# talmolab/Brax-Rodent-Run

Hardware: AMD Instinct MI355X
Metric: env-steps/sec (whole node), rodent 2048 envs/GPU (higher is better)
Workload: dtype f32

## Files before the change

### brax-rodent-run_amd/csrc/rr_api.hip

```cpp
#include "../../include/rodent_rr.h"
#include "rr_kernel.h"
#include "rr_mlp.h"
#include "rr_ppo.h"

#include <atomic>
#include <climits>
#include <cstdio>
#include <cstdlib>
#include <cstring>
#include <map>
#include <memory>
#include <mutex>
#include <string>
#include <type_traits>
#include <vector>

static thread_local std::string g_err;
static int fail(int code, const std::string& msg) { g_err = msg; return code; }
extern "C" const char* rr_last_error(void) { return g_err.c_str(); }

#define HIPCHK(x)                                                                                  \
  do {                                                                                             \
    hipError_t e_ = (x);                                                                           \
    if (e_ != hipSuccess) return fail(RR_EHIP, std::string(#x) + ": " + hipGetErrorString(e_));   \
// ... 99 lines not shown
  m->dbg_names.clear(); m->dbg_off.clear(); m->dbg_size.clear(); m->dbg_cnames.clear();
  m->stage_ok = stage_fits(d.nbody, d.nv, con_slots, k.nalias);
  if (m->dyn && d.nu > std::max(7 * d.nbody + 4, 6 * d.nv)) m->stage_ok = false;
  int g = 0;
  auto dbg = [&](const char* name, int n) { int r = g; m->dbg_names.push_back(name); m->dbg_off.push_back(g); m->dbg_size.push_back(n); g += n; return r; };
  k.g_xpos = dbg("xpos", 3 * d.nbody); k.g_xquat = dbg("xquat", 4 * d.nbody); k.g_xmat = dbg("xmat", 9 * d.nbody);
  k.g_com = dbg("subtree_com", 6); k.g_cinert = dbg("cinert", 10 * d.nbody); k.g_crb = dbg("crb", 10 * d.nbody);
  k.g_cdof = dbg("cdof", 6 * d.nv); k.g_cvel = dbg("cvel", 6 * d.nbody); k.g_cfrc = dbg("cfrc", 6 * d.nbody);
  k.g_qM = dbg("qM", d.nM); k.g_qLD = dbg("qLD", d.nM); k.g_dinv = dbg("qLDiagInv", d.nv);
  k.g_bias = dbg("qfrc_bias", d.nv); k.g_passive = dbg("qfrc_passive", d.nv); k.g_actuator = dbg("qfrc_actuator", d.nv);
  k.g_smooth = dbg("qfrc_smooth", d.nv); k.g_qacc_smooth = dbg("qacc_smooth", d.nv);
  k.g_con_dist = dbg("con_dist", d.ncon); k.g_con_pos = dbg("con_pos", 3 * d.ncon); k.g_con_frame = dbg("con_frame", 9 * d.ncon);
  k.g_con_D = dbg("con_D", d.ncon); k.g_con_aref = dbg("con_aref", 4 * d.ncon); k.g_lim = dbg("limit_pos_D_aref", 3 * d.nv);
  k.g_qacc = dbg("qacc", d.nv); k.g_qfrc_constraint = dbg("qfrc_constraint", d.nv); k.g_misc = dbg("niter_cost", 2);
  k.g_ls_iters = dbg("ls_iters", 2);
  k.g_kaok = dbg("kernarg_ok", 1);
  k.dbg_floats = g;
  for (auto& s : m->dbg_names) m->dbg_cnames.push_back(s.c_str());
  m->dims.lds_bytes = L.lds_floats * (int)sizeof(float);
  m->dims.dbg_floats = g;
  m->dims.solver = m->solver;
  m->dims.fixed_instance = select(m, F_STEP, V_PROD).fixed ? 1 : 0;
}

static void setup_replica(rr_model* m) {
  m->pair_ok = false;
  const char* sw = getenv("RR_PAIR_WAVES");
  if (sw && sw[0] == '0') return;
  static const char* need[] = {"h_dims", "h_k_slots", "h_k_body_i", "h_k_body_f", "h_k_jnt_i", "h_k_jnt_f", "h_k_dof_i", "h_k_dof_f", "h_k_act_f", "h_k_M_ij_k",
                               "h_k_body_anc", "h_k_nround", "h_k_factor3", "h_k_factor3_rows", "h_k_linv", "h_k_linv_rows", "h_k_coljob", "h_k_rowjob", "h_k_jobown",
// ... 149 lines not shown
  RRTables T_rep;
  std::vector<void*> dev_allocs;
  bool timing = false;
  std::vector<hipEvent_t> ev0, ev1;
  int npending = 0, ring_head = 0;
  double total_ms = 0;
  int64_t launches = 0;
  unsigned long long* prof = nullptr;
  const int32_t* env_map = nullptr;
  uint32_t* cost = nullptr;
  bool counted = false;
  unsigned* dyn_overflow = nullptr;
  unsigned* bad_states = nullptr;
  unsigned* progress = nullptr;
  float *env_dof_f = nullptr, *env_act_f = nullptr, *env_con_f = nullptr;
  int ls_run_repeats = 0;
  float* eval_actions = nullptr;
  bool has_env_params() const { return env_dof_f || env_act_f || env_con_f; }
};

template <typename Ptr>
static int dev_alloc(rr_batch* b, size_t bytes, Ptr* dst, const void* host = nullptr, size_t host_bytes = 0) {
  void* p = nullptr;
  HIPCHK(hipMalloc(&p, bytes));
  b->dev_allocs.push_back(p);
  if (host_bytes) HIPCHK(hipMemcpy(p, host, host_bytes, hipMemcpyHostToDevice));
  *dst = (Ptr)p;
  return RR_OK;
}
template <typename Ptr>
static int upload(rr_batch* b, const char* name, Ptr* dst) {
// ... 228 lines not shown
  if (rc) return rc;
  HIPCHK(hipSetDevice(b->device));
  const rr_model* m = b->m;
  const bool geom = io.o_cdist || io.o_cpos || io.o_cframe, params = b->has_env_params();
  if (params && io.dbg) return fail(RR_EUNSUPPORTED, "launch: no debug dump on a batch with per-env parameters (the debug instance reads the model's shared tables)");
  if (params && geom) return fail(RR_EUNSUPPORTED, "launch: no contact-geometry outputs on a batch with per-env parameters (they are served by the debug instance)");
  if (params && b->prof) return fail(RR_EUNSUPPORTED, "launch: no profile build on a batch with per-env parameters");
  Variant v = b->prof ? V_PROFILE : ((io.dbg || geom) ? V_DEBUG : (params ? V_RAND : V_PROD));
  const bool pair = m->pair_ok && v == V_PROD && !L.env && !L.out && !L.un && !b->env_map && !b->cost && m->solver != 2;
  if (pair) v = V_PAIR;
  const Instance in = select(m, L.ev ? F_EVAL : (L.ac ? F_ACTOR : (L.un ? F_UNROLL : F_STEP)), v);
  if (!in.kern) return fail(RR_EUNSUPPORTED, std::string(L.un ? "" : "launch: ") + in.why);
  if (L.un && (rc = fill_unroll(b, L, io))) return rc;
  io.env_dof_f = b->env_dof_f; io.env_act_f = b->env_act_f; io.env_con_f = b->env_con_f;
  io.prof = b->prof; io.env_map = b->env_map; io.cost = b->cost; io.dyn_overflow = b->dyn_overflow; io.bad_states = b->bad_states;
  if (v == V_DEBUG) io.ls_run_repeats = b->ls_run_repeats;
  RRDims kd = pair ? m->kd_rep : b->kd;
  kd.iterations = m->kd.iterations; kd.ls_iterations = m->kd.ls_iterations;
  if (b->timing) {
    if (b->npending == RR_TIMING_RING && (rc = collect_timing(b, false))) return rc;
    HIPCHK(hipEventRecord(b->ev0[(b->ring_head + b->npending) % RR_TIMING_RING], b->stream));
  }
  hipLaunchKernelGGL(in.kern, dim3(b->N), dim3((pair ? 2 : 1) * RR_LANES), (size_t)lds_bytes(m, v), b->stream, kd, pair ? b->T_rep : b->T, io, b->N, L.n_frames);
  HIPCHK(hipGetLastError());
  if (b->timing) {
    HIPCHK(hipEventRecord(b->ev1[(b->ring_head + b->npending) % RR_TIMING_RING], b->stream));
    b->npending += 1;
  }
  return RR_OK;
}

// ... 632 lines not shown
    *own[i] = (float*)q;
    HIPCHK(hipMemcpyAsync(q, src[i], bytes[i], hipMemcpyDeviceToDevice, b->stream));
  }
  HIPCHK(hipStreamSynchronize(b->stream));
  return RR_OK;
}

extern "C" int rr_batch_set_schedule(rr_batch* b, const int32_t* env_map, uint32_t* cost_cycles) {
  if (!b) return fail(RR_EINVAL, "rr_batch_set_schedule: null batch");
  b->env_map = env_map; b->cost = cost_cycles;
  return RR_OK;
}

extern "C" int rr_batch_set_ls_repeat_exit(rr_batch* b, int32_t enable) {
  if (!b) return fail(RR_EINVAL, "rr_batch_set_ls_repeat_exit: null batch");
  b->ls_run_repeats = enable ? 0 : 1;
  return RR_OK;
}

extern "C" int rr_batch_set_timing(rr_batch* b, int32_t enable) {
  if (!b) return fail(RR_EINVAL, "rr_batch_set_timing: null batch");
  HIPCHK(hipSetDevice(b->device));
  if (enable && b->ev0.empty()) {
    for (int i = 0; i < RR_TIMING_RING; ++i) {
      hipEvent_t a, c;
      HIPCHK(hipEventCreate(&a)); b->ev0.push_back(a);
      HIPCHK(hipEventCreate(&c)); b->ev1.push_back(c);
    }
  }
  b->timing = enable != 0;
  b->total_ms = 0; b->launches = 0; b->npending = 0; b->ring_head = 0;
// ... 11 lines not shown
```

### brax-rodent-run_amd/csrc/rr_kernel.h

```cpp
#pragma once
#include <hip/hip_runtime.h>
#include <stdint.h>
#include "rr_tanh_normal.h"

#define RR_LANES 64
#define RR_DOFI 12
#define RR_BODYI 12
#ifndef RR_WIDE
#define RR_WIDE 1
#endif
#ifndef RR_RING
#define RR_RING 6
#endif

#define RR_NPH 24
#ifndef RR_W1
#define RR_W1 2
#define RR_W2 6
#define RR_W3 12
#endif
#ifndef RR_ENV_PRIO
#define RR_ENV_PRIO 1
#endif
#ifndef RR_FACTOR_PRIO
// ... 8 lines not shown
#define RR_MINVAL 1e-15f
#define RR_MINIMP 0.0001f
#define RR_MAXIMP 0.9999f

struct RRDims {
  int nq, nv, nu, nbody, njnt, nM, ncon, dmax, nroot;
  int obs_dim, iterations, ls_iterations, nfac, nround, ninv, lmax, cmax, rmax;
  float dt, gx, gy, gz, tolerance, ls_tolerance, meaninertia;
  int o_qpos, o_qvel, o_act, o_ctrl, o_xpos, o_xquat, o_cinert, o_cdof, o_cvel,
      o_qLD, o_vec, o_x, o_arm, o_warm, o_qact, o_jlist, lds_floats;
  int o_H, o_Mp, o_anc, solver;
  int nv_scale, fac_stride, inv_stride, lds_bytes_rep;
  int nalias;
  int g_xpos, g_xquat, g_xmat, g_com, g_cinert, g_crb, g_cdof, g_cvel, g_cfrc, g_qM, g_qLD, g_dinv, g_bias, g_passive,
      g_actuator, g_smooth, g_qacc_smooth, g_con_dist, g_con_pos, g_con_frame, g_con_D, g_con_aref, g_lim, g_qacc,
      g_qfrc_constraint, g_misc, g_ls_iters, g_kaok, dbg_floats;
};

struct RRLayout {
  int o_qpos, o_qvel, o_act, o_ctrl, o_xpos, o_xquat, o_cinert, o_cdof, o_cvel, o_qLD, o_vec, o_x, o_arm, o_warm, o_qact, o_jlist, lds_floats;
  int o_H, o_Mp, o_anc;
};
constexpr int rr_imax(int a, int b) { return a > b ? a : b; }
constexpr int rr_up4(int n) { return (n + 3) & ~3; }
constexpr RRLayout rr_layout(int nq, int nv, int nu, int nbody, int nM, int ncon, bool newton = false) {
  RRLayout k{};
  int o = 0;
  k.o_qpos = o; o += rr_up4(nq);
  k.o_qvel = o; o += rr_up4(nv + 1);
  k.o_act = o; o += rr_up4(nu);
  k.o_ctrl = o; o += rr_up4(nu);
// ... 95 lines not shown
  float a_min_std;
  int a_nh;
  int a_seg, a_pad;
  unsigned* progress;
  unsigned* dyn_overflow;
  unsigned* bad_states;
  float pace_t1, pace_t2, pace_t3;
  int pace_mode;
  const float* env_dof_f;
  const float* env_act_f;
  const float* env_con_f;
  float* e_metrics;
  float* e_qpos_out;
  int mode;
  float bad_state_max;
  int ls_run_repeats;
  int num_clips;
  const int* clip;
};

struct v3 { float x, y, z; };
__device__ __forceinline__ v3 mk3(float x, float y, float z) { v3 r; r.x = x; r.y = y; r.z = z; return r; }
__device__ __forceinline__ v3 ld3(const float* p) { return mk3(p[0], p[1], p[2]); }
__device__ __forceinline__ v3 ld3(const float __attribute__((address_space(1)))* p) { return mk3(p[0], p[1], p[2]); }
__device__ __forceinline__ v3 ld3(const rr_row<float>& p) { return mk3(p[0], p[1], p[2]); }
__device__ __forceinline__ void st3(float* p, v3 a) { p[0] = a.x; p[1] = a.y; p[2] = a.z; }
__device__ __forceinline__ v3 operator+(v3 a, v3 b) { return mk3(a.x + b.x, a.y + b.y, a.z + b.z); }
__device__ __forceinline__ v3 operator-(v3 a, v3 b) { return mk3(a.x - b.x, a.y - b.y, a.z - b.z); }
__device__ __forceinline__ v3 operator*(v3 a, float s) { return mk3(a.x * s, a.y * s, a.z * s); }
__device__ __forceinline__ float dot(v3 a, v3 b) { return a.x * b.x + a.y * b.y + a.z * b.z; }
__device__ __forceinline__ v3 cross(v3 a, v3 b) { return mk3(a.y * b.z - a.z * b.y, a.z * b.x - a.x * b.z, a.x * b.y - a.y * b.x); }

__device__ __forceinline__ void quat_mul(float* r, const float* a, const float* b) {
  float w = a[0] * b[0] - a[1] * b[1] - a[2] * b[2] - a[3] * b[3];
  float x = a[0] * b[1] + a[1] * b[0] + a[2] * b[3] - a[3] * b[2];
// ... 219 lines not shown
  float dinv[NVS], dinvB[NVS];
  float Ma_warm[NVS];
  float qfrc_smooth[NVS], qacc_smooth[NVS];
  float qacc[NVS], Ma[NVS], grad[NVS], Mgrad[NVS], search[NVS], mv[NVS], qfrc_con[NVS];
  float lim_sign[NVS], lim_D[NVS], lim_aref[NVS], lim_jar[NVS], lim_jv[NVS];
  bool lim_act[NVS];
  bool con_act[NCS];
  float con_mu[NCS], con_D[NCS], con_aref[NCS][4], con_jar[NCS][4], con_jv[NCS][4];
  float con_kk[NCS], con_b[NCS];
  float con_off[NCS][3], con_fr[NCS][9];
  int con_nanc[NCS];
  float com0[3], com1[3];
  float gauss, cost, prev_cost;
  float so_tolerance, so_ls_tolerance, so_meaninertia;
  int so_iterations, so_ls_iterations, so_nv_scale;
  int dbg_ls_run_repeats = 0, dbg_ls_ran = 0, dbg_ls_left = 0;
  int work;
  unsigned long long pt_last, pt[RR_NPH];
  template <bool PROF> __device__ __forceinline__ void stamp(int i) {
    if (PROF) { const unsigned long long t = __builtin_readcyclecounter(); pt[i] += t - pt_last; pt_last = t; }
  }

  __device__ __forceinline__ DT phase_dims() const {
    if constexpr (rr_same<DT, RRDims>::value) return D;
    else return DT(load_dims());
  }
  __device__ __forceinline__ RRTables tables() const {
    if constexpr (RAND) return load_env_tables(renv, D.nv, D.nu, D.ncon);
    else return load_tables();
  }
  __device__ Wave(const DT& d, const RRTables& t, float* l)
// ... 1039 lines not shown
    for (int cs = 0; cs < NCS; ++cs) {
      out[cs][0] = out[cs][1] = out[cs][2] = out[cs][3] = 0.0f;
      if (con_act[cs]) {
        const float* w = s_buf + 6 * con_rank[cs];
        const v3 pv = mk3(w[3], w[4], w[5]) + cross(mk3(w[0], w[1], w[2]), mk3(con_off[cs][0], con_off[cs][1], con_off[cs][2]));
        const float jn_ = dot(mk3(con_fr[cs][0], con_fr[cs][1], con_fr[cs][2]), pv);
        const float j1 = dot(mk3(con_fr[cs][3], con_fr[cs][4], con_fr[cs][5]), pv);
        const float j2 = dot(mk3(con_fr[cs][6], con_fr[cs][7], con_fr[cs][8]), pv);
        const float mu = con_mu[cs];
        out[cs][0] = jn_ + mu * j1; out[cs][1] = jn_ - mu * j1; out[cs][2] = jn_ + mu * j2; out[cs][3] = jn_ - mu * j2;
      }
    }
    sync();
  }

  __device__ __forceinline__ void update_constraint() {
    float part[2] = {0.0f, 0.0f};
    float qc[NVS], cd[NVS][6];
#pragma unroll
    for (int s = 0; s < NVS; ++s) {
      const int d = lane + RR_LANES * s;
      qc[s] = 0.0f;
#pragma unroll
      for (int k = 0; k < 6; ++k) cd[s][k] = d < D.nv ? s_cdof[6 * d + k] : 0.0f;
    }
#pragma unroll
    for (int cs = 0; cs < NCS; ++cs) {
      float W[6] = {0, 0, 0, 0, 0, 0};
      bool has = false;
      if (con_act[cs]) {
        float f[4] = {0, 0, 0, 0};
#pragma unroll
        for (int k = 0; k < 4; ++k) {
          const float jr = con_jar[cs][k];
          if (jr < 0 && (!DYN || k < con_nrow[cs])) { f[k] = -con_D[cs] * jr; part[0] += con_D[cs] * jr * jr; }
        }
        const float mu = con_mu[cs];
        const float fn = f[0] + f[1] + f[2] + f[3], f1 = mu * (f[0] - f[1]), f2 = mu * (f[2] - f[3]);
        if (fn != 0.0f) {
          has = true;
          const v3 F = mk3(con_fr[cs][0], con_fr[cs][1], con_fr[cs][2]) * fn + mk3(con_fr[cs][3], con_fr[cs][4], con_fr[cs][5]) * f1 +
                       mk3(con_fr[cs][6], con_fr[cs][7], con_fr[cs][8]) * f2;
          const v3 tau = cross(mk3(con_off[cs][0], con_off[cs][1], con_off[cs][2]), F);
          W[0] = tau.x; W[1] = tau.y; W[2] = tau.z; W[3] = F.x; W[4] = F.y; W[5] = F.z;
        }
      }
      const int leaf = con_leaf[cs];
      unsigned long long mask = __ballot(has);
      while (mask) {
        const int l = __builtin_ctzll(mask);
        mask &= mask - 1;
        float w[6];
#pragma unroll
        for (int k = 0; k < 6; ++k) w[k] = __int_as_float(__builtin_amdgcn_readlane(__float_as_int(W[k]), l));
// ... 115 lines not shown
    }
    sync();
#pragma unroll
    for (int it = 0; it < NME; ++it) {
      const int ij = ment[it];
      if (ij >= 0) {
        const int i = ij & 255, j = ij >> 8;
        if (i != j) *(rr_f2*)(s_H + 2 * (lane + RR_LANES * it)) *= *(const rr_f2*)(s_buf + 2 * i);
      }
    }
    sync();
    run_levels<false, true>(TL.linv, D.ninv, delta);
    sync();
  }

  __device__ __forceinline__ void update_gradient() {
#pragma unroll
    for (int s = 0; s < NVS; ++s) { grad[s] = Ma[s] - qfrc_smooth[s] - qfrc_con[s]; Mgrad[s] = grad[s]; }
    for (int rep = 0; rep < RR_REP_SOLVE; ++rep) { float t_[NVS]; for (int s = 0; s < NVS; ++s) t_[s] = grad[s]; ldl_solve(t_); }
    if (NEWTON) {
      newton_hessian();
      newton_factor();
      ldl_solve_on(Mgrad, s_H, dinvH);
    } else {
      ldl_solve(Mgrad);
    }
  }

  __device__ __forceinline__ void ctx_create(bool at_smooth) {
    put_vec(qacc);
    jac_mul(con_jar, s_vec);
#pragma unroll
    for (int cs = 0; cs < NCS; ++cs)
#pragma unroll
      for (int k = 0; k < 4; ++k) con_jar[cs][k] -= con_aref[cs][k];
#pragma unroll
    for (int s = 0; s < NVS; ++s) lim_jar[s] = lim_sign[s] * qacc[s] - lim_aref[s];
    if (at_smooth) {
#pragma unroll
      for (int s = 0; s < NVS; ++s) Ma[s] = qfrc_smooth[s];
    } else {
#pragma unroll
      for (int s = 0; s < NVS; ++s) Ma[s] = Ma_warm[s];
    }
    cost = INFINITY; prev_cost = 0.0f;
    update_constraint();
  }

  static constexpr int KR = 4 * NCS + NVS;
  template <int NP, bool COST>
  __device__ __forceinline__ void ls_eval(const float* alpha, const float* qg, LSPoint* out, int R, const float* rjr, const float* rjv,
                                          const float* rD) {
    constexpr int NQ = COST ? 3 : 2;
    float q[NQ * NP];
#pragma unroll
    for (int i = 0; i < NQ * NP; ++i) q[i] = 0.0f;
#pragma unroll
    for (int r = 0; r < KR; ++r) {
      if (r * RR_LANES < R) {
        const float jr = rjr[r], jv = rjv[r], Dv = rD[r];
        const float q0 = 0.5f * jr * jr * Dv, q1 = jv * jr * Dv, q2 = 0.5f * jv * jv * Dv;
// ... 93 lines not shown
      ls_eval<3, false>(a3, qg, tmp3, R, rjr, rjv, rD);
      const LSPoint lo_next = tmp3[0], hi_next = tmp3[1], mid = tmp3[2];
      const bool swap_lo_next = (lo.d0 > 0) || (lo.d0 < lo_next.d0);
      if (swap_lo_next) lo = lo_next;
      const bool swap_lo_mid = (mid.d0 < 0) && (lo.d0 < mid.d0);
      if (swap_lo_mid) lo = mid;
      const bool swap_hi_next = (hi.d0 < 0) || (hi.d0 > hi_next.d0);
      if (swap_hi_next) hi = hi_next;
      const bool swap_hi_mid = (mid.d0 > 0) && (hi.d0 > mid.d0);
      if (swap_hi_mid) hi = mid;
      swap = swap_lo_next || swap_lo_mid || swap_hi_next || swap_hi_mid;
#if RR_LS_REPEAT_EXIT
      bool same = swap;
      same &= __float_as_int(lo.alpha) == __float_as_int(lo_head.alpha) && __float_as_int(lo.d0) == __float_as_int(lo_head.d0) && __float_as_int(lo.d1) == __float_as_int(lo_head.d1);
      same &= __float_as_int(hi.alpha) == __float_as_int(hi_head.alpha) && __float_as_int(hi.d0) == __float_as_int(hi_head.d0) && __float_as_int(hi.d1) == __float_as_int(hi_head.d1);
      if constexpr (DBG) same &= dbg_ls_run_repeats == 0;
      if (uni(same)) {
        if constexpr (PROF || DBG) ls_left = so_ls_iterations - 1 - it;
        it = so_ls_iterations;
        break;
      }
#endif
    }
#if RR_LS_REPEAT_EXIT
    work += 3 * (1 + (R > RR_LANES ? 1 : 0)) * (it < so_ls_iterations ? it + 1 : it);
#endif
    if constexpr (PROF) { pt[20] += (unsigned)ls_ran; pt[21] += (unsigned)ls_left; }
    if constexpr (DBG) { dbg_ls_ran += ls_ran; dbg_ls_left += ls_left; }
    {
      const float a2[2] = {lo.alpha, hi.alpha};
      LSPoint f2[2];
// ... 9 lines not shown
#pragma unroll
      for (int cs = 0; cs < NCS; ++cs)
#pragma unroll
        for (int k = 0; k < 4; ++k) con_jar[cs][k] += con_jv[cs][k] * alpha;
    }
  }

  template <bool PROF, bool DBG = false>
  __device__ __forceinline__ int solve() {
    {
      const DT Dl = phase_dims();
      so_tolerance = Dl.tolerance; so_ls_tolerance = Dl.ls_tolerance; so_meaninertia = Dl.meaninertia;
      so_iterations = Dl.iterations; so_ls_iterations = Dl.ls_iterations; so_nv_scale = Dl.nv_scale;
    }
    const float scale = 1.0f / (so_meaninertia * (float)so_nv_scale);
    float cost_smooth = 0.0f;
    bool use_smooth = false;
#pragma nounroll
    for (int ph = 0; ph < 3; ++ph) {
      if (ph == 2 && !use_smooth) break;
#pragma unroll
      for (int s = 0; s < NVS; ++s) qacc[s] = ph != 1 ? qacc_smooth[s] : (lane + RR_LANES * s < D.nv ? s_warm[lane + RR_LANES * s] : 0.0f);
      ctx_create(ph != 1);
      if (ph == 0) cost_smooth = cost;
      if (ph == 1) use_smooth = uni(!(cost < cost_smooth));
    }
    update_gradient();
#pragma unroll
    for (int s = 0; s < NVS; ++s) { search[s] = -Mgrad[s]; mv[s] = -grad[s]; }
    stamp<PROF>(8);
    int niter = 0;
    while (true) {
      const float improvement = (prev_cost - cost) * scale;
      float g2 = 0.0f;
#pragma unroll
      for (int s = 0; s < NVS; ++s) g2 += grad[s] * grad[s];
      const float gradient = sqrtf(solver_sum(g2)) * scale;
      bool done = niter >= so_iterations;
      done |= improvement < so_tolerance;
      done |= gradient < so_tolerance;
      if (uni(done)) break;
      stamp<PROF>(12);
      for (int rep = 0; rep < RR_REP_LS; ++rep) linesearch<false>();
      linesearch<PROF, DBG>();
      stamp<PROF>(9);
      float pm[NVS], gg = 0.0f;
#pragma unroll
      for (int s = 0; s < NVS; ++s) { gg += grad[s] * Mgrad[s]; pm[s] = Mgrad[s]; }
      for (int rep = 0; rep < RR_REP_UC; ++rep) { const float pc = prev_cost, c0 = cost; update_constraint(); prev_cost = pc; cost = c0; }
      update_constraint();
      stamp<PROF>(10);
      update_gradient();
      stamp<PROF>(11);
      float bt[2] = {0.0f, gg};
#pragma unroll
      for (int s = 0; s < NVS; ++s) bt[0] += grad[s] * (Mgrad[s] - pm[s]);
      solver_sum_n<2>(bt);
      const float beta = NEWTON ? 0.0f : fmaxf(0.0f, bt[0] / fmaxf(RR_MINVAL, bt[1]));
#pragma unroll
      for (int s = 0; s < NVS; ++s) { search[s] = -Mgrad[s] + beta * search[s]; mv[s] = -grad[s] + beta * mv[s]; }
      ++niter;
    }
#pragma unroll
    for (int s = 0; s < NVS; ++s) { const int d = lane + RR_LANES * s; if (d < D.nv) s_warm[d] = qacc[s]; }
    return niter;
  }

  __device__ __forceinline__ void euler() {
    float qa[NVS];
#pragma unroll
    for (int s = 0; s < NVS; ++s) qa[s] = qfrc_smooth[s] + qfrc_con[s];
    ldl_solve<true>(qa);
    const RRTables T = tables();
    const DT D = phase_dims();
#pragma unroll
// ... 213 lines not shown
```

### brax-rodent-run_amd/csrc/rr_step_body.inc

```
  static_assert(!PAIR || (!PROF && !DBG && !NEWTON && !UNROLL && !ACTOR), "PAIR: production physics instance only");
  static_assert(!DYN || (!PROF && !DBG && !NEWTON && !PAIR), "DYN: production instances only (single-step, multi-step, multi-step with the actor)");
  static_assert(!ACTOR || UNROLL, "the actor lives in the multi-step instances");
  static_assert(!EVAL || (ACTOR && !RAND && !PROF && !DBG && !NEWTON && !PAIR), "EVAL: a form of the production multi-step instance with the actor");
  extern __shared__ __attribute__((aligned(16))) float lds[];
  int env = blockIdx.x;
  if (env >= num_envs) return;
  const DT D(Dk);
  const int wrep = PAIR ? __builtin_amdgcn_readfirstlane((int)(threadIdx.x >> 6)) : 0;
  Wave<NBS, NVS, NCS, DT, NEWTON, PAIR, DYN, RAND> w(D, Tk, PAIR ? lds + wrep * (D.lds_bytes_rep >> 2) : lds);
  int lane = threadIdx.x & (RR_LANES - 1);
  if (PAIR) { w.rep = wrep; w.s_xc = lds + 2 * (D.lds_bytes_rep >> 2); }
  RRIO io = load_io();
  if (io.env_map) {
    env = __builtin_amdgcn_readfirstlane(io.env_map[env]);
    if ((unsigned)env >= (unsigned)num_envs) return;
  }
  if (RAND) w.renv = env;
  if (DBG) {
    const RRIO ref_io = io_kernarg;
    bool same = true;
    for (unsigned i = 0; i < sizeof(RRIO) / sizeof(int); ++i) same &= ((const int*)&io)[i] == ((const int*)&ref_io)[i];
    if (ref_io.dbg && lane == 0) ref_io.dbg[(size_t)env * D.dbg_floats + D.g_kaok] = same ? 1.0f : 0.0f;
    if (!same) return;
  }
// ... 134 lines not shown
      if (io.o_cinert) for (int e = lane; e < 10 * D.nbody; e += RR_LANES) io.o_cinert[(size_t)env * 10 * D.nbody + e] = w.s_cinert[e];
      if (io.o_cvel) for (int e = lane; e < 6 * D.nbody; e += RR_LANES) io.o_cvel[(size_t)env * 6 * D.nbody + e] = w.s_cvel[e];
      if (io.obs) {
        float* ob = (EVAL ? io.t_obs + ((size_t)env * 2 + ((ut + 1) & 1)) * D.obs_dim : ACTOR ? io.t_obs + rr_traj_obs(io, num_envs, env, rr_traj(io, ut).u, rr_traj(io, ut).t + 1) * D.obs_dim : io.obs + (size_t)env * D.obs_dim) + D.nq + D.nv;
        for (int i = lane; i < 10 * (D.nbody - 1); i += RR_LANES) ob[i] = w.s_cinert[10 + i];
        ob += 10 * (D.nbody - 1);
        for (int i = lane; i < 6 * (D.nbody - 1); i += RR_LANES) ob[i] = w.s_cvel[6 + i];
      }
      if (dg) for (int e = lane; e < 6 * D.nbody; e += RR_LANES) dg[D.g_cvel + e] = w.s_cvel[e];
    }
    w.backward_sweep();
    w.template stamp<PROF>(3);
    w.smooth_forces(bias, passive);
    if (dg) {
      for (int e = lane; e < 10 * D.nbody; e += RR_LANES) dg[D.g_crb + e] = w.s_crb[e];
      for (int e = lane; e < 6 * D.nbody; e += RR_LANES) dg[D.g_cfrc + e] = w.s_cfrc[e];
    }
    w.contact_jobs();
    w.env_prio();
    w.sync();
    for (int rep = 0; rep < RR_REP_MM; ++rep) w.mass_matrix();
    w.mass_matrix();
    w.template stamp<PROF>(4);
    if (dg) for (int e = lane; e < D.nM; e += RR_LANES) dg[D.g_qM + e] = w.s_qLD[2 * e];
    if (NEWTON) {
      for (int e = lane; e < D.nM + 20; e += RR_LANES) *(rr_f2*)(w.s_Mp + 2 * e) = *(const rr_f2*)(w.s_qLD + 2 * e);
      w.sync();
    }
    {
      float wv[NVS];
#pragma unroll
// ... 15 lines not shown
    w.ldl_solve(w.qacc_smooth);
    w.template stamp<PROF>(6);
    if (dg) {
#pragma unroll
      for (int s = 0; s < NVS; ++s) {
        const int d = lane + RR_LANES * s;
        if (d < D.nv) {
          dg[D.g_dinv + d] = w.dinv[s]; dg[D.g_bias + d] = bias[s]; dg[D.g_passive + d] = passive[s];
          dg[D.g_actuator + d] = w.s_qact[d]; dg[D.g_smooth + d] = w.qfrc_smooth[s];
          dg[D.g_qacc_smooth + d] = w.qacc_smooth[s];
        }
      }
    }
    w.constraint_rows(dg);
    w.template stamp<PROF>(7);
    if (DBG) { w.dbg_ls_run_repeats = io.ls_run_repeats; w.dbg_ls_ran = w.dbg_ls_left = 0; }
    niter = w.template solve<PROF, DBG>();
    w.template stamp<PROF>(12);
    if (dg) {
#pragma unroll
      for (int s = 0; s < NVS; ++s) {
        const int d = lane + RR_LANES * s;
        if (d < D.nv) { dg[D.g_qacc + d] = w.qacc[s]; dg[D.g_qfrc_constraint + d] = w.qfrc_con[s]; }
      }
      if (lane == 0) { dg[D.g_misc] = (float)niter; dg[D.g_misc + 1] = w.cost; dg[D.g_ls_iters] = (float)w.dbg_ls_ran; dg[D.g_ls_iters + 1] = (float)w.dbg_ls_left; }
    }
    if (mode & 1) w.euler();
    w.template stamp<PROF>(13);
    if (UNROLL && !last) {
      const RRIO iop = load_io();
      if (iop.progress && (iop.pace_mode & 4)) {
        unsigned seen = 0;
        if (lane == 0) seen = __hip_atomic_fetch_add(iop.progress, 1u, __ATOMIC_RELAXED, __HIP_MEMORY_SCOPE_AGENT) + 1u;
        seen = (unsigned)__builtin_amdgcn_readfirstlane((int)seen);
        const float behind = ((float)seen / (float)num_envs - (float)(ut * frames + f + 1)) / (float)frames;
        w.lag_prio = behind > iop.pace_t3 ? 3 : (behind > iop.pace_t2 ? 2 : (behind > iop.pace_t1 ? 1 : 0));
        w.lag_mode = iop.pace_mode;
      }
    }
  }
// ... 156 lines not shown
```

### brax-rodent-run_amd/rodent_amd/hip.py

```python
from __future__ import annotations

import ctypes as C
import os
from typing import Dict, Optional

import torch

_HERE = os.path.dirname(os.path.abspath(__file__))
LIB_PATH = os.environ.get("RR_LIB") or os.path.join(os.path.dirname(_HERE), "csrc", "librodent_hip.so")


class RRDims(C.Structure):
    _fields_ = [(n, C.c_int32) for n in ("nq", "nv", "nu", "na", "nbody", "njnt", "ngeom", "nM", "ncon", "nlimit",
                                         "nefc", "obs_dim", "iterations", "ls_iterations", "lds_bytes", "dbg_floats")] \
        + [("timestep", C.c_float), ("solver", C.c_int32), ("fixed_instance", C.c_int32)]


class RRState(C.Structure):
    _fields_ = [(n, C.c_void_p) for n in ("qpos", "qvel", "act", "qacc_warmstart")]


class RROutputs(C.Structure):
    _fields_ = [(n, C.c_void_p) for n in ("cinert", "cvel", "qfrc_actuator", "xpos", "xmat", "subtree_com", "debug",
                                                "contact_dist", "contact_pos", "contact_frame")]
# ... 34 lines not shown
                ("con_rows", C.c_int32), ("num_envs", C.c_int32)]


class RRDwItem(C.Structure):
    _fields_ = [(n, C.c_void_p) for n in ("delta", "act", "act_rows", "mean", "std", "delta_colsum")] + \
        [("M", C.c_int32), ("O", C.c_int32), ("I", C.c_int32), ("grad", C.c_void_p)]


class RRPpoCfg(C.Structure):
    _fields_ = [(n, C.c_float) for n in ("entropy_cost", "discounting", "reward_scaling", "gae_lambda", "clipping_epsilon", "min_std")] + \
        [("normalize_advantage", C.c_int32)]


EXPORTS = ["rr_model_load", "rr_model_dims", "rr_model_set_solver", "rr_model_set_solver_type", "rr_model_destroy", "rr_model_table", "rr_kernarg_layout", "rr_batch_create",
           "rr_batch_destroy", "rr_pipeline_init", "rr_pipeline_step", "rr_env_step", "rr_env_reset", "rr_pipeline_step_to", "rr_env_step_to", "rr_batch_contact_overflow", "rr_batch_bad_states", "rr_batch_unroll_supported", "rr_env_unroll", "rr_env_unroll_policy", "rr_batch_eval_supported", "rr_env_unroll_eval",
           "rr_compute_gae", "rr_mlp_forward", "rr_ppo_loss_workspace_bytes", "rr_ppo_loss", "rr_policy_act_workspace_bytes", "rr_policy_act", "rr_policy_sample", "rr_policy_backward_workspace_bytes", "rr_policy_backward", "rr_mlp_silu_backward_workspace_bytes", "rr_mlp_silu_backward", "rr_mlp_value_backward_workspace_bytes", "rr_mlp_policy_backward", "rr_mlp_policy_backward_workspace_bytes", "rr_mlp_value_backward", "rr_mlp_weight_grad_workspace_bytes", "rr_mlp_weight_grad", "rr_mlp_weight_grad_batch_workspace_bytes", "rr_mlp_weight_grad_batch", "rr_obs_moments_workspace_bytes", "rr_obs_moments", "rr_wrap_episode_autoreset", "rr_debug_layout", "rr_batch_set_schedule", "rr_batch_set_env_params", "rr_batch_env_params_supported", "rr_batch_set_profile", "rr_batch_set_ls_repeat_exit", "rr_batch_set_timing", "rr_batch_kernel_time", "rr_last_error"]

_lib = None


def lib():
    global _lib
    if _lib is None:
        if not os.path.exists(LIB_PATH):
            raise RuntimeError(f"{LIB_PATH} not found: run `python -c 'import __graft_entry__ as g; g.build()'`")
        L = C.CDLL(LIB_PATH)
        L.rr_last_error.restype = C.c_char_p
        L.rr_model_load.argtypes = [C.c_char_p, C.POINTER(C.c_void_p)]
        L.rr_model_dims.argtypes = [C.c_void_p, C.POINTER(RRDims)]
        L.rr_model_set_solver.argtypes = [C.c_void_p, C.c_int32, C.c_int32]
        L.rr_model_set_solver_type.argtypes = [C.c_void_p, C.c_int32]
# ... 54 lines not shown
        L.rr_mlp_weight_grad_workspace_bytes.restype = C.c_size_t
        L.rr_mlp_weight_grad.argtypes = [C.c_void_p] * 6 + [C.c_int32] * 3 + [C.c_void_p, C.c_void_p, C.c_size_t, C.c_void_p]
        L.rr_mlp_weight_grad_batch_workspace_bytes.argtypes = [C.POINTER(RRDwItem), C.c_int32]
        L.rr_mlp_weight_grad_batch_workspace_bytes.restype = C.c_size_t
        L.rr_mlp_weight_grad_batch.argtypes = [C.POINTER(RRDwItem), C.c_int32, C.c_void_p, C.c_size_t, C.c_void_p]
        L.rr_wrap_episode_autoreset.argtypes = [C.c_int32, C.c_int32, C.POINTER(C.c_void_p), C.POINTER(C.c_void_p), C.POINTER(C.c_int32)] + \
            [C.c_void_p] * 5 + [C.c_float, C.c_float, C.c_void_p]
        L.rr_obs_moments_workspace_bytes.argtypes = [C.c_int64, C.c_int32, C.c_int32]
        L.rr_obs_moments_workspace_bytes.restype = C.c_size_t
        L.rr_obs_moments.argtypes = [C.c_void_p, C.c_int64, C.c_int32, C.c_int32, C.c_int32, C.c_void_p, C.c_void_p, C.c_void_p, C.c_size_t, C.c_void_p]
        L.rr_batch_set_profile.argtypes = [C.c_void_p, C.c_void_p]
        L.rr_batch_set_schedule.argtypes = [C.c_void_p, C.c_void_p, C.c_void_p]
        L.rr_batch_set_env_params.argtypes = [C.c_void_p, C.POINTER(RREnvParams)]
        L.rr_batch_env_params_supported.argtypes = [C.c_void_p]
        L.rr_batch_set_ls_repeat_exit.argtypes = [C.c_void_p, C.c_int32]
        L.rr_batch_set_timing.argtypes = [C.c_void_p, C.c_int32]
        L.rr_batch_kernel_time.argtypes = [C.c_void_p, C.POINTER(C.c_double), C.POINTER(C.c_int64)]
        _lib = L
    return _lib


def _check(rc):
    if rc < 0:
        raise RuntimeError(f"librodent_hip: {lib().rr_last_error().decode()} (status {rc})")
    return rc


def _ptr(t: Optional[torch.Tensor], dtype=torch.float32, numel: Optional[int] = None):
    if t is None:
        return None
# ... 231 lines not shown
        _check(lib().rr_batch_set_schedule(self.h, _ptr(env_map, torch.int32, self.N), _ptr(cost, torch.int32, self.N)))

    def env_params_supported(self) -> bool:
        return _check(lib().rr_batch_env_params_supported(self.h)) == 1

    def set_env_params(self, dof_f: Optional[torch.Tensor] = None, act_f: Optional[torch.Tensor] = None, con_f: Optional[torch.Tensor] = None):
        d, N = self.dims, self.N
        for name, t, shape in (("dof_f", dof_f, (N, d.nv, 16)), ("act_f", act_f, (N, d.nu, 8)), ("con_f", con_f, (N, d.ncon, 26))):
            if t is not None and tuple(t.shape) != shape:
                raise ValueError(f"set_env_params: {name} has shape {tuple(t.shape)}, expected {shape}")
        p = RREnvParams(_ptr(dof_f), _ptr(act_f), _ptr(con_f), d.nv, d.nu, d.ncon, N)
        _check(lib().rr_batch_set_env_params(self.h, C.byref(p)))

    def set_ls_repeat_exit(self, enable: bool):
        _check(lib().rr_batch_set_ls_repeat_exit(self.h, int(enable)))

    def set_timing(self, enable: bool):
        _check(lib().rr_batch_set_timing(self.h, int(enable)))

    def kernel_time(self):
        ms, n = C.c_double(), C.c_int64()
        _check(lib().rr_batch_kernel_time(self.h, C.byref(ms), C.byref(n)))
        return ms.value, n.value


def compute_gae(truncation, termination, rewards, values, bootstrap_value, lambda_: float, discount: float):
    T, B = values.shape
    args = [t.contiguous() for t in (truncation, termination, rewards, values, bootstrap_value)]
    for t in args:
        _ptr(t)
# ... 244 lines not shown
```

### include/rodent_rr.h

```cpp
#ifndef RODENT_RR_H
#define RODENT_RR_H
#include <stddef.h>
#include <stdint.h>

#ifdef __cplusplus
extern "C" {
#endif

typedef struct rr_model rr_model;
typedef struct rr_batch rr_batch;

enum rr_status { RR_OK = 0, RR_EINVAL = -1, RR_EIO = -2, RR_EHIP = -3, RR_EUNSUPPORTED = -4 };

typedef struct rr_dims {
  int32_t nq, nv, nu, na, nbody, njnt, ngeom, nM, ncon, nlimit, nefc, obs_dim;
  int32_t iterations, ls_iterations;
  int32_t lds_bytes;
  int32_t dbg_floats;
  float timestep;
  int32_t solver;
  int32_t fixed_instance;
} rr_dims;

typedef struct rr_state {
// ... 172 lines not shown

typedef struct rr_env_params {
  const float* dof_f;
  const float* act_f;
  const float* con_f;
  int32_t dof_rows, act_rows, con_rows;
  int32_t num_envs;
} rr_env_params;
int rr_batch_set_env_params(rr_batch* b, const rr_env_params* p);
int rr_batch_env_params_supported(const rr_batch* b);

int rr_debug_layout(const rr_batch* b, const char*** names, const int32_t** offsets, const int32_t** sizes);

int rr_batch_set_ls_repeat_exit(rr_batch* b, int32_t enable);

int rr_batch_set_timing(rr_batch* b, int32_t enable);
int rr_batch_kernel_time(rr_batch* b, double* total_ms, int64_t* launches);

int rr_batch_set_profile(rr_batch* b, uint64_t* dev_cycles);

int rr_kernarg_layout(int32_t* io_offset, int32_t* io_size, int32_t* total_size);

const char* rr_last_error(void);

#ifdef __cplusplus
}
#endif
#endif
```

Before: 1.850 million.

## Trim solver warmstart: reuse smooth-phase constraint rows and defer gradient solve

```diff
diff --git a/brax-rodent-run_amd/csrc/rr_api.hip b/brax-rodent-run_amd/csrc/rr_api.hip
--- a/brax-rodent-run_amd/csrc/rr_api.hip
+++ b/brax-rodent-run_amd/csrc/rr_api.hip
@@ -137,6 +137,7 @@
   k.g_con_D = dbg("con_D", d.ncon); k.g_con_aref = dbg("con_aref", 4 * d.ncon); k.g_lim = dbg("limit_pos_D_aref", 3 * d.nv);
   k.g_qacc = dbg("qacc", d.nv); k.g_qfrc_constraint = dbg("qfrc_constraint", d.nv); k.g_misc = dbg("niter_cost", 2);
   k.g_ls_iters = dbg("ls_iters", 2);
+  k.g_solver_end = dbg("solver_end", 2);
   k.g_kaok = dbg("kernarg_ok", 1);
   k.dbg_floats = g;
   for (auto& s : m->dbg_names) m->dbg_cnames.push_back(s.c_str());
@@ -316,7 +317,7 @@
   unsigned* bad_states = nullptr;
   unsigned* progress = nullptr;
   float *env_dof_f = nullptr, *env_act_f = nullptr, *env_con_f = nullptr;
-  int ls_run_repeats = 0;
+  int dbg_flags = 0;
   float* eval_actions = nullptr;
   bool has_env_params() const { return env_dof_f || env_act_f || env_con_f; }
 };
@@ -575,7 +576,7 @@
   if (L.un && (rc = fill_unroll(b, L, io))) return rc;
   io.env_dof_f = b->env_dof_f; io.env_act_f = b->env_act_f; io.env_con_f = b->env_con_f;
   io.prof = b->prof; io.env_map = b->env_map; io.cost = b->cost; io.dyn_overflow = b->dyn_overflow; io.bad_states = b->bad_states;
-  if (v == V_DEBUG) io.ls_run_repeats = b->ls_run_repeats;
+  if (v == V_DEBUG) io.dbg_flags = b->dbg_flags;
   RRDims kd = pair ? m->kd_rep : b->kd;
   kd.iterations = m->kd.iterations; kd.ls_iterations = m->kd.ls_iterations;
   if (b->timing) {
@@ -1238,7 +1239,13 @@
 
 extern "C" int rr_batch_set_ls_repeat_exit(rr_batch* b, int32_t enable) {
   if (!b) return fail(RR_EINVAL, "rr_batch_set_ls_repeat_exit: null batch");
-  b->ls_run_repeats = enable ? 0 : 1;
+  b->dbg_flags = enable ? (b->dbg_flags & ~RR_DBG_LS_RUN_REPEATS) : (b->dbg_flags | RR_DBG_LS_RUN_REPEATS);
+  return RR_OK;
+}
+
+extern "C" int rr_batch_set_solver_trim(rr_batch* b, int32_t enable) {
+  if (!b) return fail(RR_EINVAL, "rr_batch_set_solver_trim: null batch");
+  b->dbg_flags = enable ? (b->dbg_flags & ~RR_DBG_SOLVER_UNTRIMMED) : (b->dbg_flags | RR_DBG_SOLVER_UNTRIMMED);
   return RR_OK;
 }
 
diff --git a/brax-rodent-run_amd/csrc/rr_kernel.h b/brax-rodent-run_amd/csrc/rr_kernel.h
--- a/brax-rodent-run_amd/csrc/rr_kernel.h
+++ b/brax-rodent-run_amd/csrc/rr_kernel.h
@@ -46,7 +46,7 @@
   int nalias;
   int g_xpos, g_xquat, g_xmat, g_com, g_cinert, g_crb, g_cdof, g_cvel, g_cfrc, g_qM, g_qLD, g_dinv, g_bias, g_passive,
       g_actuator, g_smooth, g_qacc_smooth, g_con_dist, g_con_pos, g_con_frame, g_con_D, g_con_aref, g_lim, g_qacc,
-      g_qfrc_constraint, g_misc, g_ls_iters, g_kaok, dbg_floats;
+      g_qfrc_constraint, g_misc, g_ls_iters, g_solver_end, g_kaok, dbg_floats;
 };
 
 struct RRLayout {
@@ -172,11 +172,13 @@
   float* e_qpos_out;
   int mode;
   float bad_state_max;
-  int ls_run_repeats;
+  int dbg_flags;
   int num_clips;
   const int* clip;
 };
 
+#define RR_DBG_LS_RUN_REPEATS 1
+#define RR_DBG_SOLVER_UNTRIMMED 2
 struct v3 { float x, y, z; };
 __device__ __forceinline__ v3 mk3(float x, float y, float z) { v3 r; r.x = x; r.y = y; r.z = z; return r; }
 __device__ __forceinline__ v3 ld3(const float* p) { return mk3(p[0], p[1], p[2]); }
@@ -426,7 +428,8 @@
   float gauss, cost, prev_cost;
   float so_tolerance, so_ls_tolerance, so_meaninertia;
   int so_iterations, so_ls_iterations, so_nv_scale;
-  int dbg_ls_run_repeats = 0, dbg_ls_ran = 0, dbg_ls_left = 0;
+  int dbg_flags = 0, dbg_ls_ran = 0, dbg_ls_left = 0;
+  int dbg_solver_end = 0;
   int work;
   unsigned long long pt_last, pt[RR_NPH];
   template <bool PROF> __device__ __forceinline__ void stamp(int i) {
@@ -1496,7 +1499,7 @@
     sync();
   }
 
-  __device__ __forceinline__ void update_constraint() {
+  __device__ __forceinline__ void update_constraint(bool walk = true) {
     float part[2] = {0.0f, 0.0f};
     float qc[NVS], cd[NVS][6];
 #pragma unroll
@@ -1519,7 +1522,7 @@
         }
         const float mu = con_mu[cs];
         const float fn = f[0] + f[1] + f[2] + f[3], f1 = mu * (f[0] - f[1]), f2 = mu * (f[2] - f[3]);
-        if (fn != 0.0f) {
+        if (walk && fn != 0.0f) {
           has = true;
           const v3 F = mk3(con_fr[cs][0], con_fr[cs][1], con_fr[cs][2]) * fn + mk3(con_fr[cs][3], con_fr[cs][4], con_fr[cs][5]) * f1 +
                        mk3(con_fr[cs][6], con_fr[cs][7], con_fr[cs][8]) * f2;
@@ -1665,9 +1668,13 @@
     sync();
   }
 
-  __device__ __forceinline__ void update_gradient() {
-#pragma unroll
-    for (int s = 0; s < NVS; ++s) { grad[s] = Ma[s] - qfrc_smooth[s] - qfrc_con[s]; Mgrad[s] = grad[s]; }
+  __device__ __forceinline__ void form_gradient() {
+#pragma unroll
+    for (int s = 0; s < NVS; ++s) grad[s] = Ma[s] - qfrc_smooth[s] - qfrc_con[s];
+  }
+  __device__ __forceinline__ void solve_gradient() {
+#pragma unroll
+    for (int s = 0; s < NVS; ++s) Mgrad[s] = grad[s];
     for (int rep = 0; rep < RR_REP_SOLVE; ++rep) { float t_[NVS]; for (int s = 0; s < NVS; ++s) t_[s] = grad[s]; ldl_solve(t_); }
     if (NEWTON) {
       newton_hessian();
@@ -1678,15 +1685,32 @@
     }
   }
 
-  __device__ __forceinline__ void ctx_create(bool at_smooth) {
-    put_vec(qacc);
-    jac_mul(con_jar, s_vec);
-#pragma unroll
-    for (int cs = 0; cs < NCS; ++cs)
-#pragma unroll
-      for (int k = 0; k < 4; ++k) con_jar[cs][k] -= con_aref[cs][k];
-#pragma unroll
-    for (int s = 0; s < NVS; ++s) lim_jar[s] = lim_sign[s] * qacc[s] - lim_aref[s];
+  __device__ __forceinline__ void direction(int niter, const float* pm, float gg) {
+    if (niter == 0) {
+#pragma unroll
+      for (int s = 0; s < NVS; ++s) { search[s] = -Mgrad[s]; mv[s] = -grad[s]; }
+    } else {
+      float bt[2] = {0.0f, gg};
+#pragma unroll
+      for (int s = 0; s < NVS; ++s) bt[0] += grad[s] * (Mgrad[s] - pm[s]);
+      solver_sum_n<2>(bt);
+      const float beta = NEWTON ? 0.0f : fmaxf(0.0f, bt[0] / fmaxf(RR_MINVAL, bt[1]));
+#pragma unroll
+      for (int s = 0; s < NVS; ++s) { search[s] = -Mgrad[s] + beta * search[s]; mv[s] = -grad[s] + beta * mv[s]; }
+    }
+  }
+
+  __device__ __forceinline__ void ctx_create(bool at_smooth, bool rows_kept, bool walk) {
+    if (!rows_kept) {
+      put_vec(qacc);
+      jac_mul(con_jar, s_vec);
+#pragma unroll
+      for (int cs = 0; cs < NCS; ++cs)
+#pragma unroll
+        for (int k = 0; k < 4; ++k) con_jar[cs][k] -= con_aref[cs][k];
+#pragma unroll
+      for (int s = 0; s < NVS; ++s) lim_jar[s] = lim_sign[s] * qacc[s] - lim_aref[s];
+    }
     if (at_smooth) {
 #pragma unroll
       for (int s = 0; s < NVS; ++s) Ma[s] = qfrc_smooth[s];
@@ -1695,7 +1719,7 @@
       for (int s = 0; s < NVS; ++s) Ma[s] = Ma_warm[s];
     }
     cost = INFINITY; prev_cost = 0.0f;
-    update_constraint();
+    update_constraint(walk);
   }
 
   static constexpr int KR = 4 * NCS + NVS;
@@ -1819,7 +1843,7 @@
       bool same = swap;
       same &= __float_as_int(lo.alpha) == __float_as_int(lo_head.alpha) && __float_as_int(lo.d0) == __float_as_int(lo_head.d0) && __float_as_int(lo.d1) == __float_as_int(lo_head.d1);
       same &= __float_as_int(hi.alpha) == __float_as_int(hi_head.alpha) && __float_as_int(hi.d0) == __float_as_int(hi_head.d0) && __float_as_int(hi.d1) == __float_as_int(hi_head.d1);
-      if constexpr (DBG) same &= dbg_ls_run_repeats == 0;
+      if constexpr (DBG) same &= (dbg_flags & RR_DBG_LS_RUN_REPEATS) == 0;
       if (uni(same)) {
         if constexpr (PROF || DBG) ls_left = so_ls_iterations - 1 - it;
         it = so_ls_iterations;
@@ -1859,23 +1883,50 @@
       so_iterations = Dl.iterations; so_ls_iterations = Dl.ls_iterations; so_nv_scale = Dl.nv_scale;
     }
     const float scale = 1.0f / (so_meaninertia * (float)so_nv_scale);
+    const bool untrimmed = DBG && (dbg_flags & RR_DBG_SOLVER_UNTRIMMED) != 0;
     float cost_smooth = 0.0f;
     bool use_smooth = false;
+    float jar0[NCS][4], ljar0[NVS];
+#pragma unroll
+    for (int cs = 0; cs < NCS; ++cs)
+#pragma unroll
+      for (int k = 0; k < 4; ++k) jar0[cs][k] = 0.0f;
+#pragma unroll
+    for (int s = 0; s < NVS; ++s) ljar0[s] = 0.0f;
 #pragma nounroll
     for (int ph = 0; ph < 3; ++ph) {
       if (ph == 2 && !use_smooth) break;
 #pragma unroll
       for (int s = 0; s < NVS; ++s) qacc[s] = ph != 1 ? qacc_smooth[s] : (lane + RR_LANES * s < D.nv ? s_warm[lane + RR_LANES * s] : 0.0f);
-      ctx_create(ph != 1);
-      if (ph == 0) cost_smooth = cost;
+      const bool rows_kept = ph == 2 && !untrimmed;
+      if (rows_kept) {
+#pragma unroll
+        for (int cs = 0; cs < NCS; ++cs)
+#pragma unroll
+          for (int k = 0; k < 4; ++k) con_jar[cs][k] = jar0[cs][k];
+#pragma unroll
+        for (int s = 0; s < NVS; ++s) lim_jar[s] = ljar0[s];
+      }
+      ctx_create(ph != 1, rows_kept, ph != 0 || untrimmed);
+      if (ph == 0) {
+        cost_smooth = cost;
+#pragma unroll
+        for (int cs = 0; cs < NCS; ++cs)
+#pragma unroll
+          for (int k = 0; k < 4; ++k) jar0[cs][k] = con_jar[cs][k];
+#pragma unroll
+        for (int s = 0; s < NVS; ++s) ljar0[s] = lim_jar[s];
+      }
       if (ph == 1) use_smooth = uni(!(cost < cost_smooth));
     }
-    update_gradient();
-#pragma unroll
-    for (int s = 0; s < NVS; ++s) { search[s] = -Mgrad[s]; mv[s] = -grad[s]; }
-    stamp<PROF>(8);
+    if constexpr (DBG) dbg_solver_end = use_smooth ? 1 : 0;
+    form_gradient();
     int niter = 0;
+    float pm[NVS], gg = 0.0f;
+#pragma unroll
+    for (int s = 0; s < NVS; ++s) pm[s] = 0.0f;
     while (true) {
+      if (untrimmed) { solve_gradient(); direction(niter, pm, gg); }
       const float improvement = (prev_cost - cost) * scale;
       float g2 = 0.0f;
 #pragma unroll
@@ -1884,26 +1935,27 @@
       bool done = niter >= so_iterations;
       done |= improvement < so_tolerance;
       done |= gradient < so_tolerance;
-      if (uni(done)) break;
-      stamp<PROF>(12);
+      if (uni(done)) {
+        if constexpr (DBG) dbg_solver_end |= (niter >= so_iterations ? 2 : 0) | (uni(improvement < so_tolerance) ? 4 : 0) | (uni(gradient < so_tolerance) ? 8 : 0);
+        break;
+      }
+      if constexpr (PROF) { if (niter) stamp<PROF>(12); }
+      if (!untrimmed) {
+        solve_gradient();
+        if constexpr (PROF) { if (niter) stamp<PROF>(11); }
+        direction(niter, pm, gg);
+      }
+      if constexpr (PROF) { if (niter) stamp<PROF>(12); else stamp<PROF>(8); }
       for (int rep = 0; rep < RR_REP_LS; ++rep) linesearch<false>();
       linesearch<PROF, DBG>();
       stamp<PROF>(9);
-      float pm[NVS], gg = 0.0f;
+      gg = 0.0f;
 #pragma unroll
       for (int s = 0; s < NVS; ++s) { gg += grad[s] * Mgrad[s]; pm[s] = Mgrad[s]; }
       for (int rep = 0; rep < RR_REP_UC; ++rep) { const float pc = prev_cost, c0 = cost; update_constraint(); prev_cost = pc; cost = c0; }
       update_constraint();
       stamp<PROF>(10);
-      update_gradient();
-      stamp<PROF>(11);
-      float bt[2] = {0.0f, gg};
-#pragma unroll
-      for (int s = 0; s < NVS; ++s) bt[0] += grad[s] * (Mgrad[s] - pm[s]);
-      solver_sum_n<2>(bt);
-      const float beta = NEWTON ? 0.0f : fmaxf(0.0f, bt[0] / fmaxf(RR_MINVAL, bt[1]));
-#pragma unroll
-      for (int s = 0; s < NVS; ++s) { search[s] = -Mgrad[s] + beta * search[s]; mv[s] = -grad[s] + beta * mv[s]; }
+      form_gradient();
       ++niter;
     }
 #pragma unroll
diff --git a/brax-rodent-run_amd/csrc/rr_step_body.inc b/brax-rodent-run_amd/csrc/rr_step_body.inc
--- a/brax-rodent-run_amd/csrc/rr_step_body.inc
+++ b/brax-rodent-run_amd/csrc/rr_step_body.inc
@@ -172,7 +172,7 @@
     w.smooth_forces(bias, passive);
     if (dg) {
       for (int e = lane; e < 10 * D.nbody; e += RR_LANES) dg[D.g_crb + e] = w.s_crb[e];
-      for (int e = lane; e < 6 * D.nbody; e += RR_LANES) dg[D.g_cfrc + e] = w.s_cfrc[e];
+      for (int e = lane; e < 6 * D.nbody; e += RR_LANES) dg[D.g_cfrc + e] = e < 6 ? 0.0f : w.s_cfrc[e];
     }
     w.contact_jobs();
     w.env_prio();
@@ -218,7 +218,7 @@
     }
     w.constraint_rows(dg);
     w.template stamp<PROF>(7);
-    if (DBG) { w.dbg_ls_run_repeats = io.ls_run_repeats; w.dbg_ls_ran = w.dbg_ls_left = 0; }
+    if (DBG) { w.dbg_flags = io.dbg_flags; w.dbg_ls_ran = w.dbg_ls_left = 0; }
     niter = w.template solve<PROF, DBG>();
     w.template stamp<PROF>(12);
     if (dg) {
@@ -227,7 +227,11 @@
         const int d = lane + RR_LANES * s;
         if (d < D.nv) { dg[D.g_qacc + d] = w.qacc[s]; dg[D.g_qfrc_constraint + d] = w.qfrc_con[s]; }
       }
-      if (lane == 0) { dg[D.g_misc] = (float)niter; dg[D.g_misc + 1] = w.cost; dg[D.g_ls_iters] = (float)w.dbg_ls_ran; dg[D.g_ls_iters + 1] = (float)w.dbg_ls_left; }
+      if (lane == 0) {
+        dg[D.g_misc] = (float)niter; dg[D.g_misc + 1] = w.cost;
+        dg[D.g_ls_iters] = (float)w.dbg_ls_ran; dg[D.g_ls_iters + 1] = (float)w.dbg_ls_left;
+        dg[D.g_solver_end] = (float)(w.dbg_solver_end & 1); dg[D.g_solver_end + 1] = (float)(w.dbg_solver_end >> 1);
+      }
     }
     if (mode & 1) w.euler();
     w.template stamp<PROF>(13);
diff --git a/brax-rodent-run_amd/rodent_amd/hip.py b/brax-rodent-run_amd/rodent_amd/hip.py
--- a/brax-rodent-run_amd/rodent_amd/hip.py
+++ b/brax-rodent-run_amd/rodent_amd/hip.py
@@ -72,7 +72,7 @@
 
 EXPORTS = ["rr_model_load", "rr_model_dims", "rr_model_set_solver", "rr_model_set_solver_type", "rr_model_destroy", "rr_model_table", "rr_kernarg_layout", "rr_batch_create",
            "rr_batch_destroy", "rr_pipeline_init", "rr_pipeline_step", "rr_env_step", "rr_env_reset", "rr_pipeline_step_to", "rr_env_step_to", "rr_batch_contact_overflow", "rr_batch_bad_states", "rr_batch_unroll_supported", "rr_env_unroll", "rr_env_unroll_policy", "rr_batch_eval_supported", "rr_env_unroll_eval",
-           "rr_compute_gae", "rr_mlp_forward", "rr_ppo_loss_workspace_bytes", "rr_ppo_loss", "rr_policy_act_workspace_bytes", "rr_policy_act", "rr_policy_sample", "rr_policy_backward_workspace_bytes", "rr_policy_backward", "rr_mlp_silu_backward_workspace_bytes", "rr_mlp_silu_backward", "rr_mlp_value_backward_workspace_bytes", "rr_mlp_policy_backward", "rr_mlp_policy_backward_workspace_bytes", "rr_mlp_value_backward", "rr_mlp_weight_grad_workspace_bytes", "rr_mlp_weight_grad", "rr_mlp_weight_grad_batch_workspace_bytes", "rr_mlp_weight_grad_batch", "rr_obs_moments_workspace_bytes", "rr_obs_moments", "rr_wrap_episode_autoreset", "rr_debug_layout", "rr_batch_set_schedule", "rr_batch_set_env_params", "rr_batch_env_params_supported", "rr_batch_set_profile", "rr_batch_set_ls_repeat_exit", "rr_batch_set_timing", "rr_batch_kernel_time", "rr_last_error"]
+           "rr_compute_gae", "rr_mlp_forward", "rr_ppo_loss_workspace_bytes", "rr_ppo_loss", "rr_policy_act_workspace_bytes", "rr_policy_act", "rr_policy_sample", "rr_policy_backward_workspace_bytes", "rr_policy_backward", "rr_mlp_silu_backward_workspace_bytes", "rr_mlp_silu_backward", "rr_mlp_value_backward_workspace_bytes", "rr_mlp_policy_backward", "rr_mlp_policy_backward_workspace_bytes", "rr_mlp_value_backward", "rr_mlp_weight_grad_workspace_bytes", "rr_mlp_weight_grad", "rr_mlp_weight_grad_batch_workspace_bytes", "rr_mlp_weight_grad_batch", "rr_obs_moments_workspace_bytes", "rr_obs_moments", "rr_wrap_episode_autoreset", "rr_debug_layout", "rr_batch_set_schedule", "rr_batch_set_env_params", "rr_batch_env_params_supported", "rr_batch_set_profile", "rr_batch_set_ls_repeat_exit", "rr_batch_set_solver_trim", "rr_batch_set_timing", "rr_batch_kernel_time", "rr_last_error"]
 
 _lib = None
 
@@ -157,6 +157,7 @@
         L.rr_batch_set_env_params.argtypes = [C.c_void_p, C.POINTER(RREnvParams)]
         L.rr_batch_env_params_supported.argtypes = [C.c_void_p]
         L.rr_batch_set_ls_repeat_exit.argtypes = [C.c_void_p, C.c_int32]
+        L.rr_batch_set_solver_trim.argtypes = [C.c_void_p, C.c_int32]
         L.rr_batch_set_timing.argtypes = [C.c_void_p, C.c_int32]
         L.rr_batch_kernel_time.argtypes = [C.c_void_p, C.POINTER(C.c_double), C.POINTER(C.c_int64)]
         _lib = L
@@ -418,6 +419,9 @@
 
     def set_ls_repeat_exit(self, enable: bool):
         _check(lib().rr_batch_set_ls_repeat_exit(self.h, int(enable)))
+
+    def set_solver_trim(self, enable: bool):
+        _check(lib().rr_batch_set_solver_trim(self.h, int(enable)))
 
     def set_timing(self, enable: bool):
         _check(lib().rr_batch_set_timing(self.h, int(enable)))
diff --git a/include/rodent_rr.h b/include/rodent_rr.h
--- a/include/rodent_rr.h
+++ b/include/rodent_rr.h
@@ -210,6 +210,8 @@
 
 int rr_batch_set_ls_repeat_exit(rr_batch* b, int32_t enable);
 
+int rr_batch_set_solver_trim(rr_batch* b, int32_t enable);
+
 int rr_batch_set_timing(rr_batch* b, int32_t enable);
 int rr_batch_kernel_time(rr_batch* b, double* total_ms, int64_t* launches);
 
```

New measurement: 1.898 million, median of 6. 1.03x the previous value.
